# wavelab/libwave

Measured on AMD Instinct MI355X. Metric: point-cloud registrations/sec (1M<->1M pts, ICP), higher is better.
Workload: dtype f32

## Files before the change

### libwave_amd/csrc/wm_nn.hip

```cpp
#include "wm_nn_scan.hpp"

namespace wm {

template <int STATS, bool BAL, bool COST = false>
__global__ void __launch_bounds__(64) __attribute__((amdgpu_waves_per_eu(5, 5)))
    k_nn_grid(const LevelsDev lv, const float4 *__restrict__ src, unsigned n,
              IcpDevState *__restrict__ st, float thr_d2, unsigned long long *__restrict__ keys,
              float4 *__restrict__ match_pt, const float4 *__restrict__ tgt_orig,
              float r_light_cells, float lane_lf, float coop_lf, float r0_cells, unsigned chunk_sz,
              double *__restrict__ partials, unsigned *__restrict__ cost_out,
              unsigned long long *__restrict__ phase_out, long long *__restrict__ bins, float rmax) {
    const unsigned lane = threadIdx.x & 63u;
    const unsigned row_c = xcd_remap_chunked(blockIdx.x, max(chunk_sz, 1u)), row_e = xcd_remap(blockIdx.x, gridDim.x);
    const unsigned row = chunk_sz ? row_c : row_e;
    const unsigned i = row * 64u + lane;
    const bool active = i < n;
    const unsigned ic = min(i, n - 1u);
    const float4 p_e = src[ic];
    const unsigned long long prev_e = keys[ic];
    const float4 tp_e = match_pt[ic];
    const NnState S = nn_state(st);
    const int L = lv.n;
    float hl[kMaxLevels];
#pragma unroll
    for (int k = 0; k < kMaxLevels; ++k) hl[k] = lv.g[k].h;
    asm volatile("" ::WM_NN_STATE_OPERANDS(S), "v"(p_e.x), "v"(p_e.y), "v"(p_e.z), "v"(prev_e), "v"(tp_e.x), "v"(tp_e.y),
                 "v"(tp_e.z), "v"(tp_e.w));
    asm volatile("" ::"s"(L), "s"(hl[0]), "s"(hl[1]), "s"(hl[2]), "s"(hl[3]), "s"(hl[4]), "s"(hl[5]), "s"(r_light_cells),
                 "s"(lane_lf), "s"(r0_cells), "s"(thr_d2), "s"(rmax));
    if (S.done) return;
    unsigned cost = 0;
    unsigned long long prof[3] = {0ull, 0ull, 0ull};
    const unsigned long long prof_start = COST ? clock64() : 0ull;
    __shared__ uint2 s_runs[BAL ? 1 : kRowChunk * 64];
    __shared__ BalHolder<BAL> s_hold;
    const int L_levels = L;
    const float h0 = hl[0];
    const float r_light = r_light_cells * h0;
    const bool have_prev = S.have_prev != 0;
    float qx = 0.f, qy = 0.f, qz = 0.f, r = 0.f;
    float bqx = 0.f, bqy = 0.f, bqz = 0.f;
    unsigned long long best = make_key(thr_d2, kNoIdx);
    unsigned long long seeded = best;
    bool heavy = false;
    bool mine = active;
    unsigned long long prev = ~0ull;
    float4 tp = make_float4(0.f, 0.f, 0.f, 0.f);
    if (active) {
        if (have_prev) {
            prev = prev_e;
            tp = tp_e;
        }
        xform(S.Tf, p_e, qx, qy, qz);
        if (S.slab_on && !(qx >= S.slab_lo && qx < S.slab_hi)) mine = false;
    }
    if (mine) {
        r = r0_cells * h0;
        if (prev != ~0ull) {
            const unsigned pidx = (unsigned) prev;
            r = rmax;
            if (pidx != kNoIdx) {
                const float d2b = canon_d2(qx, qy, qz, tp);
                if (d2b <= thr_d2) {
                    best = seeded = make_key(d2b, pidx);
                    bqx = tp.x;
                    bqy = tp.y;
                    bqz = tp.z;
                    r = fmaxf(__builtin_amdgcn_sqrtf(d2b) * 1.0001f + 1e-6f, 0.05f * h0);
                }
            }
        }
        r = fminf(r, rmax);
        heavy = r > r_light;
    }
    const unsigned long long prof_pro = COST ? clock64() : 0ull;
    if constexpr (BAL) {
        BalLds &L = s_hold.v;
        L.q[lane] = make_float4(qx, qy, qz, 0.f);
        L.seeded[lane] = seeded;
        L.bq[0][lane] = bqx;
        L.bq[1][lane] = bqy;
        L.bq[2][lane] = bqz;
        asm volatile("" ::: "memory");
        bool live = mine && !heavy;
        const bool allow_layered = true;
        for (int pass = 0; pass < 32 && __ballot(live) != 0ull; ++pass) {
            const int l = nn_level_for(hl, L_levels, lane_lf, r);
            const unsigned long long lv_mask = __ballot(live);
            const int l0 = __builtin_amdgcn_readlane(l, __ffsll((long long) lv_mask) - 1);
            float margin;
            if (__ballot(live && l != l0) == 0ull) {
                const GridDev g = lv.g[l0];
                best = scan_box_bal<COST, kBalRowChunk>(g, live, qx, qy, qz, r, best, &margin, L, lane, allow_layered, g.pts, cost, prof);
            } else {
                const GridDev g = lv.g[l];
                L.base[lane] = (unsigned long long) g.pts;
                best = scan_box_bal<COST, kBalRowChunk>(g, live, qx, qy, qz, r, best, &margin, L, lane, allow_layered, nullptr, cost, prof);
            }
            if (live) {
                if constexpr (COST) cost += 1u << 24;
                const float bd2 = __uint_as_float((unsigned) (best >> 32));
                if (nn_certified(margin, bd2, thr_d2)) {
                    live = false;
                } else {
                    r = nn_grow_radius(best, bd2, r, rmax);
                    heavy = r > r_light;
                    live = !heavy;
                }
            }
        }
    } else if (mine) {
        for (int pass = 0; !heavy && pass < 32; ++pass) {
            const int l = nn_level_for(hl, L_levels, lane_lf, r);
            const GridDev g = lv.g[l];
            float margin;
            best = scan_box<COST>(g, qx, qy, qz, r, best, &margin, s_runs, lane, have_prev, cost);
            if constexpr (COST) cost += 1u << 24;
            const float bd2 = __uint_as_float((unsigned) (best >> 32));
            if (nn_certified(margin, bd2, thr_d2)) break;
            r = nn_grow_radius(best, bd2, r, rmax);
            heavy = r > r_light;
        }
    }
    const unsigned long long prof_pass = COST ? clock64() : 0ull;
    unsigned long long todo = __ballot(heavy);
    const unsigned n_heavy = __popcll(todo);
    float seed = 0.f;
    while (todo) {
        const int sl = __ffsll((long long) todo) - 1;
        todo &= todo - 1;
        const float ux = rl_f(qx, sl), uy = rl_f(qy, sl), uz = rl_f(qz, sl);
        float ur = rl_f(r, sl);
        unsigned long long ub = ((unsigned long long) rl_u((unsigned) (best >> 32), sl) << 32) |
                                rl_u((unsigned) best, sl);
        if ((unsigned) ub == kNoIdx && seed > ur) ur = fminf(seed, rmax);
        for (int pass = 0; pass < 64; ++pass) {
            const int l = nn_level_for(hl, L_levels, coop_lf, ur);
            const GridDev g = lv.g[l];
            float margin;
            ub = coop_scan_box(g, ux, uy, uz, ur, ub, lane, &margin);
            const float bd2 = __uint_as_float((unsigned) (ub >> 32));
            if (nn_certified(margin, bd2, thr_d2)) break;
            if (ur >= rmax) break;
            ur = nn_grow_radius(ub, bd2, ur, rmax);
        }
        seed = ((unsigned) ub != kNoIdx) ? 1.25f * sqrtf(__uint_as_float((unsigned) (ub >> 32))) : ur;
        if ((int) lane == sl) best = ub;
    }
    const unsigned lane_e = __builtin_amdgcn_mbcnt_hi(~0u, __builtin_amdgcn_mbcnt_lo(~0u, 0u));
    const unsigned i_e = BAL ? row * 64u + lane_e : i;
    if constexpr (BAL) {
        asm volatile("" ::: "memory");
        BalLds &L = s_hold.v;
        seeded = L.seeded[lane_e];
        bqx = L.bq[0][lane_e];
        bqy = L.bq[1][lane_e];
        bqz = L.bq[2][lane_e];
    }
    if (mine) {
        st_u64(&keys[i_e], best);
        if (best != seeded && (unsigned) best != kNoIdx) {
            const f4v c = ((gp_f4) tgt_orig)[(unsigned) best];
            bqx = c.x;
            bqy = c.y;
            bqz = c.z;
        }
        if (!(best == seeded && (unsigned) best != kNoIdx))
            st_f4(&match_pt[i_e], bqx, bqy, bqz, __uint_as_float((unsigned) best));
    }
    if (lane == 0 && n_heavy) atomicAdd(&st->queue_count[1], n_heavy);
    const unsigned long long prof_store = COST ? clock64() : 0ull;
    if constexpr (COST) {
        if (active) cost_out[i_e] = mine ? (cost | (heavy ? 0x80000000u : 0u)) : 0u;
    }
    if constexpr (STATS >= 0) {
        double a[kAcc];
        icp_terms<STATS>(a, mine, (unsigned) best != kNoIdx, qx, qy, qz, bqx, bqy, bqz,
                         __uint_as_float((unsigned) (best >> 32)),
                         (unsigned) best != (unsigned) seeded && (i_e & st->changed_mask) == 0u);
        acc_halve<kAcc, 32>(a, lane);
        const int comp = acc_comp_of_lane(lane);
        if (comp >= 0) {
            if (bins) bins_add(bins, row % (unsigned) kBinCount, (unsigned) comp, a[0]);
            else st_f64(&partials[(size_t) row * kAcc + comp], a[0]);
        }
    }
    if constexpr (COST) {
        if (lane_e == 0 && phase_out) {
            const unsigned long long t_end = clock64();
            atomicAdd(&phase_out[0], prof[0]);
            atomicAdd(&phase_out[1], prof[1]);
            atomicAdd(&phase_out[2], prof[2]);
            atomicAdd(&phase_out[3], prof_pro - prof_start);
            atomicAdd(&phase_out[4], prof_pass - prof_pro);
            atomicAdd(&phase_out[5], prof_store - prof_pass);
            atomicAdd(&phase_out[6], t_end - prof_store);
            atomicAdd(&phase_out[7], 1ull);
        }
    }
}

constexpr int kBruteTile = 1024;

__global__ void __launch_bounds__(kBlock) k_init_keys(unsigned long long *keys, unsigned n,
                                                       const IcpDevState *st, float thr_d2) {
    if (st->done) return;
    const unsigned i = blockIdx.x * kBlock + threadIdx.x;
    if (i < n) keys[i] = make_key(thr_d2, kNoIdx);
}

__global__ void __launch_bounds__(kBlock)
    k_nn_brute(const float4 *__restrict__ tgt, unsigned m, const float4 *__restrict__ src,
               unsigned n, const IcpDevState *__restrict__ st, float thr_d2,
               unsigned long long *__restrict__ keys) {
    if (st->done) return;
    __shared__ float4 tile[kBruteTile];
    const unsigned i = blockIdx.x * kBlock + threadIdx.x;
    const unsigned per = (m + gridDim.y - 1) / gridDim.y;
    const unsigned m0 = blockIdx.y * per, m1 = min(m0 + per, m);
    float qx = 0, qy = 0, qz = 0;
    if (i < n) xform(st->Tf, src[i], qx, qy, qz);
    const bool mine = !(st->slab_on && !(qx >= st->slab_lo && qx < st->slab_hi));
    unsigned long long best = make_key(thr_d2, kNoIdx);
    for (unsigned t0 = m0; t0 < m1; t0 += kBruteTile) {
        const unsigned cnt = min((unsigned) kBruteTile, m1 - t0);
        __syncthreads();
        for (unsigned k = threadIdx.x; k < cnt; k += kBlock) tile[k] = tgt[t0 + k];
        __syncthreads();
        for (unsigned k = 0; k < cnt; ++k) {
            const float4 t = tile[k];
            const unsigned long long key = make_key(canon_d2(qx, qy, qz, t), __float_as_uint(t.w));
            best = key < best ? key : best;
        }
    }
    if (i < n && mine && best < make_key(thr_d2, kNoIdx)) atomicMin(&keys[i], best);
}

__global__ void __launch_bounds__(kBlock)
    k_fill_match(const unsigned long long *__restrict__ keys, unsigned n,
                 const float4 *__restrict__ tgt, const IcpDevState *__restrict__ st,
                 float4 *__restrict__ match_pt) {
    if (st->done) return;
    const unsigned i = blockIdx.x * kBlock + threadIdx.x;
    if (i >= n) return;
    const unsigned idx = (unsigned) keys[i];
    match_pt[i] = idx == kNoIdx ? make_float4(0.f, 0.f, 0.f, __uint_as_float(kNoIdx)) : tgt[idx];
}

static float threshold_below(double max_corr, bool strict) {
    const double m2 = max_corr * max_corr;
    if (!(m2 < 3.0e38)) return 3.0e38f;
    float f = (float) m2;
    if (strict ? (double) f >= m2 : (double) f > m2) f = nextafterf(f, 0.0f);
    return f;
}
float threshold_d2(double max_corr) { return threshold_below(max_corr, false); }
float threshold_d2_strict(double max_corr) { return threshold_below(max_corr, true); }

int nn_sums_target(wm_ctx *ctx, int stats_mode, bool use_bins, unsigned blocks, long long **bins, unsigned *rows_out) {
    *bins = nullptr;
    if (stats_mode >= 0 && use_bins) {
        if (!ctx->bins.p) return WM_ERR_STATE;
        *bins = ctx->bins.as<long long>();
    } else if (stats_mode >= 0) {
        WM_HIP(ctx, ctx->partials.reserve((size_t) blocks * kAcc * sizeof(double)));
        if (rows_out) *rows_out = blocks;
    }
    return WM_OK;
}

template <int STATS, bool BAL, bool COST = false>
static void launch_nn_grid_t(wm_ctx *ctx, unsigned blocks, float thr_d2, unsigned xcd_chunk, long long *bins = nullptr) {
    hipLaunchKernelGGL(HIP_KERNEL_NAME(k_nn_grid<STATS, BAL, COST>), dim3(blocks), dim3(64), 0, ctx->stream,
                       ctx->levels_dev, ctx->src_sorted.as<float4>(), (unsigned) ctx->n_src,
                       ctx->d_state.as<IcpDevState>(), thr_d2, ctx->keys.as<unsigned long long>(),
                       ctx->match_pt.as<float4>(), ctx->tgt_orig.as<float4>(), ctx->tune_r_light,
                       ctx->tune_lane_lf, ctx->tune_coop_lf, ctx->tune_r0, xcd_chunk, ctx->partials.as<double>(),
                       ctx->cost_log.p ? ctx->cost_log.as<unsigned>() + (size_t) ctx->cost_log_iter * ctx->n_src : nullptr,
                       ctx->phase_log.p ? ctx->phase_log.as<unsigned long long>() + 8 * (size_t) ctx->cost_log_iter : nullptr, bins,
                       sqrtf(thr_d2) * 1.0001f + 1e-6f);
}

int launch_nn_grid(wm_ctx *ctx, float thr_d2, hipEvent_t ev0, hipEvent_t ev1, hipEvent_t ev2,
                   int stats_mode, unsigned *rows_out, bool use_bins) {
    const unsigned n = (unsigned) ctx->n_src;
    if (rows_out) *rows_out = 0;
    if (n == 0) return WM_OK;
    unsigned blocks = (n + 63u) / 64u;
    blocks = (blocks + 7u) & ~7u;
    unsigned xcd_chunk = 0;
    if (ctx->tune_xcd_chunk > 0 && blocks >= 32u * (unsigned) ctx->tune_xcd_chunk) {
        xcd_chunk = (unsigned) ctx->tune_xcd_chunk;
        const unsigned m = 8u * xcd_chunk;
        blocks = (blocks + m - 1u) / m * m;
    }
    long long *bins = nullptr;
    const int rc = nn_sums_target(ctx, stats_mode, use_bins, blocks, &bins, rows_out);
    if (rc != WM_OK) return rc;
    const bool bal = ctx->tune_nn_balanced && ctx->n_tgt_input < (1u << 26) - 8u;
    if (ev0) WM_HIP(ctx, hipEventRecord(ev0, ctx->stream));
    if (stats_mode == WM_ICP_SVD && ctx->cost_log.p && ctx->cost_log_iter < ctx->cost_log_cap) {
        if (bal) launch_nn_grid_t<WM_ICP_SVD, true, true>(ctx, blocks, thr_d2, xcd_chunk, bins);
        else launch_nn_grid_t<WM_ICP_SVD, false, true>(ctx, blocks, thr_d2, xcd_chunk, bins);
        ctx->cost_log_iter++;
    } else if (stats_mode < 0) {
        if (bal) launch_nn_grid_t<-1, true>(ctx, blocks, thr_d2, xcd_chunk);
        else launch_nn_grid_t<-1, false>(ctx, blocks, thr_d2, xcd_chunk);
    } else if (stats_mode == WM_ICP_SVD) {
        if (bal) launch_nn_grid_t<WM_ICP_SVD, true>(ctx, blocks, thr_d2, xcd_chunk, bins);
        else launch_nn_grid_t<WM_ICP_SVD, false>(ctx, blocks, thr_d2, xcd_chunk, bins);
    } else {
        if (bal) launch_nn_grid_t<WM_ICP_GN6, true>(ctx, blocks, thr_d2, xcd_chunk, bins);
        else launch_nn_grid_t<WM_ICP_GN6, false>(ctx, blocks, thr_d2, xcd_chunk, bins);
    }
    if (ev1) WM_HIP(ctx, hipEventRecord(ev1, ctx->stream));
    if (ev2) WM_HIP(ctx, hipEventRecord(ev2, ctx->stream));
    WM_HIP(ctx, hipGetLastError());
    return WM_OK;
}

int launch_nn_brute(wm_ctx *ctx, float thr_d2, hipEvent_t ev0, hipEvent_t ev1) {
    const unsigned n = (unsigned) ctx->n_src, m = (unsigned) ctx->n_tgt_input;
    if (n == 0) return WM_OK;
    const IcpDevState *st = ctx->d_state.as<IcpDevState>();
    unsigned long long *keys = ctx->keys.as<unsigned long long>();
    const unsigned bx = (n + kBlock - 1) / kBlock;
    unsigned splits = 1;
    if (m > 0) {
        splits = (2048 + bx - 1) / bx;
        const unsigned max_splits = (m + kBruteTile - 1) / kBruteTile;
        if (splits > max_splits) splits = max_splits;
        if (splits < 1) splits = 1;
    }
    if (ev0) WM_HIP(ctx, hipEventRecord(ev0, ctx->stream));
    hipLaunchKernelGGL(k_init_keys, dim3(bx), dim3(kBlock), 0, ctx->stream, keys, n, st, thr_d2);
    if (m > 0)
        hipLaunchKernelGGL(k_nn_brute, dim3(bx, splits), dim3(kBlock), 0, ctx->stream,
                           ctx->tgt_orig.as<float4>(), m, ctx->src_sorted.as<float4>(), n, st,
                           thr_d2, keys);
    hipLaunchKernelGGL(k_fill_match, dim3(bx), dim3(kBlock), 0, ctx->stream, keys, n,
                       ctx->tgt_orig.as<float4>(), st, ctx->match_pt.as<float4>());
    if (ev1) WM_HIP(ctx, hipEventRecord(ev1, ctx->stream));
    WM_HIP(ctx, hipGetLastError());
    return WM_OK;
}

}
```

### libwave_amd/csrc/wm_nn_scan.hpp

```cpp
#pragma once
#include "wm_internal.hpp"
#include "wm_icp_step.hpp"
#include "wm_bins.hpp"
#include "wm_wave.hpp"
#include "wm_zigzag.hpp"

namespace wm {

__device__ __forceinline__ unsigned long long make_key(float d2, unsigned idx) {
    return ((unsigned long long) __float_as_uint(d2) << 32) | idx;
}

__device__ __forceinline__ float canon_d2(float qx, float qy, float qz, const float4 &t) {
    const float dx = qx - t.x, dy = qy - t.y, dz = qz - t.z;
    return __fadd_rn(__fadd_rn(__fmul_rn(dx, dx), __fmul_rn(dy, dy)), __fmul_rn(dz, dz));
}

__device__ __forceinline__ void xform(const float *T, const float4 &p, float &x, float &y,
                                      float &z) {
    x = __fadd_rn(__fadd_rn(__fadd_rn(__fmul_rn(T[0], p.x), __fmul_rn(T[1], p.y)),
                            __fmul_rn(T[2], p.z)), T[3]);
    y = __fadd_rn(__fadd_rn(__fadd_rn(__fmul_rn(T[4], p.x), __fmul_rn(T[5], p.y)),
                            __fmul_rn(T[6], p.z)), T[7]);
    z = __fadd_rn(__fadd_rn(__fadd_rn(__fmul_rn(T[8], p.x), __fmul_rn(T[9], p.y)),
                            __fmul_rn(T[10], p.z)), T[11]);
}

__device__ __forceinline__ unsigned xcd_remap(unsigned b, unsigned nblocks) {
    const unsigned per = (nblocks + 7u) / 8u;
    return (b & 7u) * per + (b >> 3);
}
__device__ __forceinline__ unsigned xcd_remap_chunked(unsigned b, unsigned S) {
    const unsigned x = b & 7u, l = b >> 3;
    const unsigned chunk = l / S;
    return (chunk * 8u + x) * S + (l - chunk * S);
}

struct NnState {
    float Tf[12];
    int done, have_prev, slab_on;
    float slab_lo, slab_hi;
    unsigned changed_mask;
    float step_disp;
};
__device__ __forceinline__ NnState nn_state(const IcpDevState *st) {
    NnState s;
#pragma unroll
    for (int k = 0; k < 12; ++k) s.Tf[k] = st->Tf[k];
    s.done = st->done;
    s.have_prev = st->have_prev;
    s.slab_on = st->slab_on;
    s.slab_lo = st->slab_lo;
    s.slab_hi = st->slab_hi;
    s.changed_mask = st->changed_mask;
    s.step_disp = st->step_disp;
    return s;
}
#define WM_NN_STATE_OPERANDS(s)                                                                                              \
    "s"((s).Tf[0]), "s"((s).Tf[1]), "s"((s).Tf[2]), "s"((s).Tf[3]), "s"((s).Tf[4]), "s"((s).Tf[5]), "s"((s).Tf[6]),           \
        "s"((s).Tf[7]), "s"((s).Tf[8]), "s"((s).Tf[9]), "s"((s).Tf[10]), "s"((s).Tf[11]), "s"((s).done), "s"((s).have_prev), \
        "s"((s).slab_on), "s"((s).slab_lo), "s"((s).slab_hi)

typedef float f4v __attribute__((ext_vector_type(4)));
typedef const __attribute__((address_space(1))) f4v *gp_f4;
typedef const __attribute__((address_space(1))) unsigned *gp_u32;
__device__ __forceinline__ float4 ldp(const float4 *p, size_t j) {
    const f4v v = ((gp_f4) p)[j];
    return make_float4(v.x, v.y, v.z, v.w);
}
__device__ __forceinline__ unsigned ldc(const unsigned *p, size_t j) { return ((gp_u32) p)[j]; }
__device__ __forceinline__ void st_f4(float4 *p, float x, float y, float z, float w) {
    f4v v = {x, y, z, w};
    __builtin_nontemporal_store(v, (f4v *) p);
}
__device__ __forceinline__ void st_u64(unsigned long long *p, unsigned long long v) { __builtin_nontemporal_store(v, p); }
__device__ __forceinline__ void st_f64(double *p, double v) { __builtin_nontemporal_store(v, p); }
__device__ __forceinline__ float canon_d2v(float qx, float qy, float qz, const f4v &t) {
    return canon_d2(qx, qy, qz, make_float4(t.x, t.y, t.z, t.w));
}

__device__ __forceinline__ unsigned long long scan_run(const float4 *__restrict__ pts, unsigned s,
                                                       unsigned e, float qx, float qy, float qz,
                                                       unsigned long long best) {
    for (unsigned j = s; j < e; j += 4) {
        const gp_f4 p = (gp_f4) pts + j;
        const f4v t0 = p[0], t1 = p[1], t2 = p[2], t3 = p[3];
        const unsigned long long k0 = make_key(canon_d2v(qx, qy, qz, t0), __float_as_uint(t0.w));
        const unsigned long long k1 = make_key(canon_d2v(qx, qy, qz, t1), __float_as_uint(t1.w));
        const unsigned long long k2 = make_key(canon_d2v(qx, qy, qz, t2), __float_as_uint(t2.w));
        const unsigned long long k3 = make_key(canon_d2v(qx, qy, qz, t3), __float_as_uint(t3.w));
        const unsigned long long a = k0 < k1 ? k0 : k1, b = k2 < k3 ? k2 : k3;
        const unsigned long long m = a < b ? a : b;
        best = m < best ? m : best;
    }
    return best;
}

constexpr int kRowChunk = 6;
constexpr int kLayeredRows = 18;
template <bool COST>
__device__ __forceinline__ unsigned long long scan_box(const GridDev &g, float qx, float qy,
                                                       float qz, float r, unsigned long long best,
                                                       float *margin, uint2 *runs, unsigned lane,
                                                       bool allow_layered, unsigned &cost) {
    const float big = 4.0e6f;
    const float fx = fminf(fmaxf((qx - g.ox) * g.inv_h, -big), big);
    const float fy = fminf(fmaxf((qy - g.oy) * g.inv_h, -big), big);
    const float fz = fminf(fmaxf((qz - g.oz) * g.inv_h, -big), big);
    const float rc = r * g.inv_h + g.slack;
    const int x0 = (int) floorf(fx - rc), x1 = (int) floorf(fx + rc);
    const int y0 = (int) floorf(fy - rc), y1 = (int) floorf(fy + rc);
    const int z0 = (int) floorf(fz - rc), z1 = (int) floorf(fz + rc);
    const float mx = fminf(fx - (float) x0, (float) (x1 + 1) - fx);
    const float my = fminf(fy - (float) y0, (float) (y1 + 1) - fy);
    const float mz = fminf(fz - (float) z0, (float) (z1 + 1) - fz);
    *margin = (fminf(mx, fminf(my, mz)) - g.slack) * g.h;
    const int xa = max(x0, 0), xb = min(x1, g.nx - 1);
    const int ya = max(y0, 0), yb = min(y1, g.ny - 1);
    const int za = max(z0, 0), zb = min(z1, g.nz - 1);
    if (xa > xb || ya > yb || za > zb) return best;
    auto lookup_and_walk = [&](const unsigned (&a0)[kRowChunk], const unsigned (&a1)[kRowChunk]) {
        unsigned rs[kRowChunk], re[kRowChunk];
#pragma unroll
        for (int u = 0; u < kRowChunk; ++u) {
            rs[u] = ldc(g.cell_start, a0[u]);
            re[u] = ldc(g.cell_start, a1[u]);
        }
        unsigned cnt = 0;
        if constexpr (COST) cost += 1u << 16;
#pragma unroll
        for (int u = 0; u < kRowChunk; ++u)
            if (re[u] > rs[u]) runs[cnt++ * 64u + lane] = make_uint2(rs[u], re[u]);
        unsigned idx = 0, j = 0, e = 0;
        if (cnt) {
            const uint2 run = runs[lane];
            j = run.x;
            e = run.y;
        }
        while (j < e) {
            const gp_f4 p = (gp_f4) g.pts + j;
            const f4v t0 = p[0], t1 = p[1], t2 = p[2], t3 = p[3];
            const unsigned long long k0 = make_key(canon_d2v(qx, qy, qz, t0), __float_as_uint(t0.w));
            const unsigned long long k1 = make_key(canon_d2v(qx, qy, qz, t1), __float_as_uint(t1.w));
            const unsigned long long k2 = make_key(canon_d2v(qx, qy, qz, t2), __float_as_uint(t2.w));
            const unsigned long long k3 = make_key(canon_d2v(qx, qy, qz, t3), __float_as_uint(t3.w));
            const unsigned long long a = k0 < k1 ? k0 : k1, b = k2 < k3 ? k2 : k3;
            const unsigned long long m = a < b ? a : b;
            best = m < best ? m : best;
            j += 4;
            if constexpr (COST) cost += 1u;
            if (j >= e && ++idx < cnt) {
                const uint2 run = runs[idx * 64u + lane];
                j = run.x;
                e = run.y;
            }
        }
    };
    const bool layered =
        allow_layered && __popcll(__ballot((yb - ya + 1) * (zb - za + 1) > kLayeredRows)) >= 8;
    if (layered) {
        for (int kz = 0;; ++kz) {
            const int zz = za + kz;
            const bool zact = zz <= zb;
            if (__ballot(zact) == 0ull) break;
            const float Rb =
                __builtin_amdgcn_sqrtf(__uint_as_float((unsigned) (best >> 32))) * g.inv_h * 1.00001f;
            const float lim = Rb + g.slack;
            const float lim2 = lim * lim, c0 = Rb * Rb + 2.f * g.slack * lim;
            const float rz = fmaxf(fmaxf((float) zz - fz, fz - (float) (zz + 1)), 0.f);
            const float rz2 = rz * rz;
            const float hy = __builtin_amdgcn_sqrtf(fmaxf(lim2 - rz2, 0.f)) * 1.00001f;
            const bool zin = zact && !(rz2 > lim2);
            const int yl = zin ? max(ya, __float2int_rd(fy - hy)) : 1;
            const int yh = zin ? min(yb, __float2int_rd(fy + hy)) : 0;
            const unsigned basez = (unsigned) zz * g.ny * g.nx;
            for (int y0 = yl; __ballot(y0 <= yh) != 0ull; y0 += kRowChunk) {
                unsigned a0[kRowChunk], a1[kRowChunk];
#pragma unroll
                for (int u = 0; u < kRowChunk; ++u) {
                    const int yy = y0 + u;
                    const float yf = (float) yy;
                    const float ry = fmaxf(fmaxf(yf - fy, fy - (yf + 1.f)), 0.f);
                    const float rho2 = ry * ry + rz2;
                    const float hx = __builtin_amdgcn_sqrtf(fmaxf(c0 - rho2, 0.f)) * 1.00001f + g.slack;
                    const int xl = max(xa, __float2int_rd(fx - hx)), xh = min(xb, __float2int_rd(fx + hx));
                    const bool ok = yy <= yh && !(rho2 > lim2) && xl <= xh;
                    const unsigned base = basez + (unsigned) yy * g.nx;
                    a0[u] = ok ? base + xl : 0u;
                    a1[u] = ok ? base + xh + 1 : 0u;
                }
                lookup_and_walk(a0, a1);
            }
        }
        return best;
    }
    int yy = ya, zz = za;
    while (zz <= zb) {
        const float Rb =
            __builtin_amdgcn_sqrtf(__uint_as_float((unsigned) (best >> 32))) * g.inv_h * 1.00001f;
        const float lim = Rb + g.slack;
        const float lim2 = lim * lim, c0 = Rb * Rb + 2.f * g.slack * lim;
        unsigned a0[kRowChunk], a1[kRowChunk];
#pragma unroll
        for (int u = 0; u < kRowChunk; ++u) {
            const float ry = fmaxf(fmaxf((float) yy - fy, fy - (float) (yy + 1)), 0.f);
            const float rz = fmaxf(fmaxf((float) zz - fz, fz - (float) (zz + 1)), 0.f);
            const float rho2 = ry * ry + rz * rz;
            const float hx = __builtin_amdgcn_sqrtf(fmaxf(c0 - rho2, 0.f)) * 1.00001f + g.slack;
            const int xl = max(xa, __float2int_rd(fx - hx)), xh = min(xb, __float2int_rd(fx + hx));
            const bool ok = zz <= zb && !(rho2 > lim2) && xl <= xh;
            const unsigned base = ((unsigned) zz * g.ny + yy) * g.nx;
            a0[u] = ok ? base + xl : 0u;
            a1[u] = ok ? base + xh + 1 : 0u;
            const bool wrap = yy >= yb;
            yy = wrap ? ya : yy + 1;
            zz += wrap;
        }
        lookup_and_walk(a0, a1);
    }
    return best;
}

__device__ __forceinline__ unsigned long long scan_run_bound(const float4 *__restrict__ pts, unsigned s, unsigned e,
                                                             float qx, float qy, float qz, unsigned long long best,
                                                             unsigned &second) {
    for (unsigned j = s; j < e; j += 4) {
        const gp_f4 p = (gp_f4) pts + j;
        const f4v t[4] = {p[0], p[1], p[2], p[3]};
#pragma unroll
        for (int u = 0; u < 4; ++u) {
            const unsigned long long k = make_key(canon_d2v(qx, qy, qz, t[u]), __float_as_uint(t[u].w));
            if (k < best) {
                second = min(second, (unsigned) (best >> 32));
                best = k;
            } else if (k != best) {
                second = min(second, (unsigned) (k >> 32));
            }
        }
    }
    return best;
}

__device__ __forceinline__ unsigned long long wave_min_u64(unsigned long long v) {
#pragma unroll
    for (int off = 32; off > 0; off >>= 1) {
        const unsigned long long o = __shfl_xor(v, off);
        v = o < v ? o : v;
    }
    return v;
}

__device__ __forceinline__ float rl_f(float v, int lane) {
    return __int_as_float(__builtin_amdgcn_readlane(__float_as_int(v), lane));
}
__device__ __forceinline__ unsigned rl_u(unsigned v, int lane) {
    return (unsigned) __builtin_amdgcn_readlane((int) v, lane);
}

constexpr int kBalCap = 1024;
constexpr int kBalRowChunk = 3;
struct BalLds {
    unsigned items[kBalCap + 1];
    float4 q[64];
    unsigned long long base[64];
    unsigned long long best[64];
    unsigned long long seeded[64];
    float bq[3][64];
};

__device__ __forceinline__ unsigned wave_incl_scan(unsigned v) {
    v += (unsigned) __builtin_amdgcn_update_dpp(0, (int) v, 0x111, 0xf, 0xf, true);
    v += (unsigned) __builtin_amdgcn_update_dpp(0, (int) v, 0x112, 0xf, 0xf, true);
    v += (unsigned) __builtin_amdgcn_update_dpp(0, (int) v, 0x114, 0xf, 0xf, true);
    v += (unsigned) __builtin_amdgcn_update_dpp(0, (int) v, 0x118, 0xf, 0xf, true);
    v += (unsigned) __builtin_amdgcn_update_dpp(0, (int) v, 0x142, 0xa, 0xf, false);
    v += (unsigned) __builtin_amdgcn_update_dpp(0, (int) v, 0x143, 0xc, 0xf, false);
    return v;
}

template <bool B>
struct BalHolder {
    BalLds v;
};
template <>
struct BalHolder<false> {
    int unused;
};

struct Bound {
    unsigned second;
    float pad;
    unsigned *lds;
    float4 *win;
    bool ok;
    __device__ __forceinline__ float prune_r(unsigned long long best) const {
        const float b = __builtin_amdgcn_sqrtf(__uint_as_float((unsigned) (best >> 32))) * 1.00001f + pad;
        return fminf(b, __builtin_amdgcn_sqrtf(__uint_as_float(second)) * 1.00001f);
    }
};

template <bool BOUND>
__device__ __forceinline__ void pooled_rounds(BalLds &L, const unsigned *items, unsigned T, unsigned lane,
                                              const float4 *ubase, Bound *bnd) {
    for (unsigned k0 = 0; k0 < T; k0 += 64u) {
        const unsigned k = k0 + lane;
        if (k < T) {
            const unsigned it = items[k];
            const unsigned owner = it >> 26, j = it & 0x3FFFFFFu;
            const float4 q = L.q[owner];
            const gp_f4 p = (gp_f4) (ubase ? ubase : (const float4 *) L.base[owner]) + j;
            const f4v t0 = p[0], t1 = p[1], t2 = p[2], t3 = p[3];
            const float d0 = canon_d2v(q.x, q.y, q.z, t0), d1 = canon_d2v(q.x, q.y, q.z, t1);
            const float d2 = canon_d2v(q.x, q.y, q.z, t2), d3 = canon_d2v(q.x, q.y, q.z, t3);
            const unsigned m = min(min(__float_as_uint(d0), __float_as_uint(d1)), min(__float_as_uint(d2), __float_as_uint(d3)));
            if (m <= __float_as_uint(q.w)) {
                const unsigned long long k0_ = make_key(d0, __float_as_uint(t0.w)), k1_ = make_key(d1, __float_as_uint(t1.w));
                const unsigned long long k2_ = make_key(d2, __float_as_uint(t2.w)), k3_ = make_key(d3, __float_as_uint(t3.w));
                const unsigned long long a = k0_ < k1_ ? k0_ : k1_, b = k2_ < k3_ ? k2_ : k3_;
                if constexpr (BOUND) {
                    const unsigned long long mn = a < b ? a : b;
                    const unsigned u0 = __float_as_uint(d0), u1 = __float_as_uint(d1), u2 = __float_as_uint(d2),
                                   u3 = __float_as_uint(d3);
                    const unsigned lo01 = min(u0, u1), hi01 = max(u0, u1), lo23 = min(u2, u3), hi23 = max(u2, u3);
                    const unsigned sec = min(max(lo01, lo23), min(hi01, hi23));
                    const unsigned long long old = atomicMin(&L.best[owner], mn);
                    unsigned push = sec;
                    if (old != mn) push = min(push, (unsigned) ((old > mn ? old : mn) >> 32));
                    atomicMin(&bnd->lds[owner], push);
                    if (old > mn && bnd->win) {
                        const f4v c = mn == k0_ ? t0 : (mn == k1_ ? t1 : (mn == k2_ ? t2 : t3));
                        bnd->win[owner] = make_float4(c.x, c.y, c.z, c.w);
                    }
                } else {
                    atomicMin(&L.best[owner], a < b ? a : b);
                }
            }
        }
    }
}

template <bool COST, int RC, bool BOUND = false>
__device__ __forceinline__ void balanced_walk(BalLds &L, const unsigned (&rs)[RC],
                                              const unsigned (&re)[RC], unsigned lane,
                                              const float4 *pts, const float4 *ubase, float qx, float qy,
                                              float qz, unsigned long long &best, unsigned &cost,
                                              unsigned long long *prof, Bound *bnd = nullptr) {
    const unsigned long long prof_t0 = COST ? clock64() : 0ull;
    unsigned len[RC], t = 0, longest = 0;
#pragma unroll
    for (int u = 0; u < RC; ++u) {
        len[u] = (unsigned) max((int) (re[u] - rs[u]), 0);
        t += (len[u] + 3u) >> 2;
        longest = max(longest, len[u]);
    }
    const unsigned incl = wave_incl_scan(t);
    const unsigned T = rl_u(incl, 63);
    if (T == 0u) return;
    if constexpr (COST) cost += t;
    if (T > (unsigned) kBalCap) {
        if constexpr (BOUND) {
#pragma unroll
            for (int u = 0; u < RC; ++u) best = scan_run_bound(pts, rs[u], re[u], qx, qy, qz, best, bnd->second);
        } else {
#pragma unroll
            for (int u = 0; u < RC; ++u) best = scan_run(pts, rs[u], re[u], qx, qy, qz, best);
        }
        return;
    }
    unsigned off = incl - t;
    const unsigned tag = lane << 26;
    if (__ballot(longest > 8u) == 0ull) {
#pragma unroll
        for (int u = 0; u < RC; ++u) {
            L.items[len[u] > 0u ? off : (unsigned) kBalCap] = tag | rs[u];
            L.items[len[u] > 4u ? off + 1u : (unsigned) kBalCap] = tag | (rs[u] + 4u);
            off += (len[u] + 3u) >> 2;
        }
    } else {
#pragma unroll
        for (int u = 0; u < RC; ++u)
            for (unsigned j = rs[u]; j < re[u]; j += 4u) L.items[off++] = tag | j;
    }
    L.best[lane] = best;
    if constexpr (BOUND) {
        const float pr = bnd->prune_r(best);
        bnd->lds[lane] = bnd->second;
        reinterpret_cast<unsigned *>(&L.q[lane])[3] = __float_as_uint(pr * pr);
    } else {
        reinterpret_cast<unsigned *>(&L.q[lane])[3] = (unsigned) (best >> 32);
    }
    __builtin_amdgcn_wave_barrier();
    pooled_rounds<BOUND>(L, L.items, T, lane, ubase, bnd);
    __builtin_amdgcn_wave_barrier();
    best = L.best[lane];
    if constexpr (BOUND) bnd->second = bnd->lds[lane];
    if constexpr (COST) {
        prof[0] += clock64() - prof_t0;
        prof[1] += (T + 63u) / 64u;
        prof[2] += 1;
    }
}

template <bool COST, int RC, bool BOUND = false>
__device__ __forceinline__ unsigned long long scan_box_bal(const GridDev &g, bool live, float qx, float qy,
                                                           float qz, float r, unsigned long long best,
                                                           float *margin, BalLds &L, unsigned lane,
                                                           bool allow_layered, const float4 *ubase,
                                                           unsigned &cost, unsigned long long *prof, Bound *bnd = nullptr) {
    const float big = 4.0e6f;
    const float fx = fminf(fmaxf((qx - g.ox) * g.inv_h, -big), big);
    const float fy = fminf(fmaxf((qy - g.oy) * g.inv_h, -big), big);
    const float fz = fminf(fmaxf((qz - g.oz) * g.inv_h, -big), big);
    const float rc = r * g.inv_h + g.slack;
    const int x0 = (int) floorf(fx - rc), x1 = (int) floorf(fx + rc);
    const int y0 = (int) floorf(fy - rc), y1 = (int) floorf(fy + rc);
    const int z0 = (int) floorf(fz - rc), z1 = (int) floorf(fz + rc);
    const float mx = fminf(fx - (float) x0, (float) (x1 + 1) - fx);
    const float my = fminf(fy - (float) y0, (float) (y1 + 1) - fy);
    const float mz = fminf(fz - (float) z0, (float) (z1 + 1) - fz);
    *margin = (fminf(mx, fminf(my, mz)) - g.slack) * g.h;
    const int xa = max(x0, 0), xb = min(x1, g.nx - 1);
    const int ya = max(y0, 0), yb = min(y1, g.ny - 1);
    const int za = max(z0, 0), zb = min(z1, g.nz - 1);
    const bool has = live && !(xa > xb || ya > yb || za > zb);
    auto lookup_and_walk = [&](const unsigned (&a0)[RC], const unsigned (&a1)[RC]) {
        unsigned rs[RC], re[RC];
#pragma unroll
        for (int u = 0; u < RC; ++u) {
            rs[u] = ldc(g.cell_start, a0[u]);
            re[u] = ldc(g.cell_start, a1[u]);
        }
        if constexpr (COST) cost += has ? 1u << 16 : 0u;
        balanced_walk<COST, RC, BOUND>(L, rs, re, lane, g.pts, ubase, qx, qy, qz, best, cost, prof, bnd);
    };
    auto ball_r = [&]() -> float {
        if constexpr (BOUND) return bnd->prune_r(best) * g.inv_h * 1.00001f;
        else return __builtin_amdgcn_sqrtf(__uint_as_float((unsigned) (best >> 32))) * g.inv_h * 1.00001f;
    };
    const bool layered =
        allow_layered && __popcll(__ballot(has && (yb - ya + 1) * (zb - za + 1) > kLayeredRows)) >= 8;
    if (layered) {
        const int zq = min(max(__float2int_rd(fz), za), zb);
        for (int kz = 0;; ++kz) {
            const float Rb = ball_r();
            const float lim = Rb + g.slack;
            const float lim2 = lim * lim;
            const float dz = zigzag_remaining(kz, za, zq, zb, 0.f);
            const bool zact = has && kz <= zb - za && !(dz * dz > lim2);
            if (__ballot(zact) == 0ull) break;
            const int zz = zigzag_coord(kz, za, zq, zb);
            const float rz = fmaxf(fmaxf((float) zz - fz, fz - (float) (zz + 1)), 0.f);
            const float rz2 = rz * rz;
            const float hy = __builtin_amdgcn_sqrtf(fmaxf(lim2 - rz2, 0.f)) * 1.00001f;
            const bool zin = zact && !(rz2 > lim2);
            const int yl = zin ? max(ya, __float2int_rd(fy - hy)) : 1;
            const int yh = zin ? min(yb, __float2int_rd(fy + hy)) : 0;
            const int yc = min(max(__float2int_rd(fy), yl), yh);
            const unsigned basez = (unsigned) zz * g.ny * g.nx;
            for (int ky = 0;; ky += RC) {
                const float Rc = ball_r();
                const float limc = Rc + g.slack;
                const float limc2 = limc * limc, c0 = Rc * Rc + 2.f * g.slack * limc;
                const float dy = zigzag_remaining(ky, yl, yc, yh, 0.f);
                const bool yact = ky <= yh - yl && !(dy * dy + rz2 > limc2);
                if (__ballot(yact) == 0ull) break;
                unsigned a0[RC], a1[RC];
#pragma unroll
                for (int u = 0; u < RC; ++u) {
                    const int yy = zigzag_coord(ky + u, yl, yc, yh);
                    const float yf = (float) yy;
                    const float ry = fmaxf(fmaxf(yf - fy, fy - (yf + 1.f)), 0.f);
                    const float rho2 = ry * ry + rz2;
                    const float hx = __builtin_amdgcn_sqrtf(fmaxf(c0 - rho2, 0.f)) * 1.00001f + g.slack;
                    const int xl = max(xa, __float2int_rd(fx - hx)), xh = min(xb, __float2int_rd(fx + hx));
                    const bool ok = yact && ky + u <= yh - yl && !(rho2 > limc2) && xl <= xh;
                    const unsigned base = basez + (unsigned) yy * g.nx;
                    a0[u] = ok ? base + xl : 0u;
                    a1[u] = ok ? base + xh + 1 : 0u;
                }
                lookup_and_walk(a0, a1);
            }
        }
        return best;
    }
    int yy = ya, zz = has ? za : zb + 1;
    while (__ballot(zz <= zb) != 0ull) {
        const float Rb = ball_r();
        const float lim = Rb + g.slack;
        const float lim2 = lim * lim, c0 = Rb * Rb + 2.f * g.slack * lim;
        unsigned a0[RC], a1[RC];
#pragma unroll
        for (int u = 0; u < RC; ++u) {
            const float ry = fmaxf(fmaxf((float) yy - fy, fy - (float) (yy + 1)), 0.f);
            const float rz = fmaxf(fmaxf((float) zz - fz, fz - (float) (zz + 1)), 0.f);
            const float rho2 = ry * ry + rz * rz;
            const float hx = __builtin_amdgcn_sqrtf(fmaxf(c0 - rho2, 0.f)) * 1.00001f + g.slack;
            const int xl = max(xa, __float2int_rd(fx - hx)), xh = min(xb, __float2int_rd(fx + hx));
            const bool ok = zz <= zb && !(rho2 > lim2) && xl <= xh;
            const unsigned base = ((unsigned) zz * g.ny + yy) * g.nx;
            a0[u] = ok ? base + xl : 0u;
            a1[u] = ok ? base + xh + 1 : 0u;
            const bool wrap = yy >= yb;
            yy = wrap ? ya : yy + 1;
            zz += (wrap && zz <= zb) ? 1 : 0;
        }
        lookup_and_walk(a0, a1);
    }
    return best;
}

constexpr unsigned kRowPool = 128, kRowsPerLane = 16, kRowTrips = 512;
struct RowLds {
    unsigned trips[kRowTrips];
    unsigned map[kRowPool];
    int box[5][64];
};
static_assert(sizeof(RowLds) <= sizeof(unsigned) * (kBalCap + 1), "RowLds overlays BalLds::items");

__device__ __forceinline__ bool scan_box_rows(const GridDev &g, bool live, float qx, float qy, float qz, float r,
                                              unsigned long long &best, float *margin, BalLds &L, unsigned lane,
                                              Bound *bnd) {
    const float big = 4.0e6f;
    const float fx = fminf(fmaxf((qx - g.ox) * g.inv_h, -big), big);
    const float fy = fminf(fmaxf((qy - g.oy) * g.inv_h, -big), big);
    const float fz = fminf(fmaxf((qz - g.oz) * g.inv_h, -big), big);
    const float rc = r * g.inv_h + g.slack;
    const int x0 = (int) floorf(fx - rc), x1 = (int) floorf(fx + rc);
    const int y0 = (int) floorf(fy - rc), y1 = (int) floorf(fy + rc);
    const int z0 = (int) floorf(fz - rc), z1 = (int) floorf(fz + rc);
    const int xa = max(x0, 0), xb = min(x1, g.nx - 1);
    const int ya = max(y0, 0), yb = min(y1, g.ny - 1);
    const int za = max(z0, 0), zb = min(z1, g.nz - 1);
    const bool has = live && !(xa > xb || ya > yb || za > zb);
    const int wy = yb - ya + 1;
    const unsigned nrows = has ? (unsigned) (wy * (zb - za + 1)) : 0u;
    const unsigned incl = wave_incl_scan(nrows);
    const unsigned R = rl_u(incl, 63);
    if (R > kRowPool || __ballot(nrows > kRowsPerLane) != 0ull) return false;
    {
        const float mx = fminf(fx - (float) x0, (float) (x1 + 1) - fx);
        const float my = fminf(fy - (float) y0, (float) (y1 + 1) - fy);
        const float mz = fminf(fz - (float) z0, (float) (z1 + 1) - fz);
        *margin = (fminf(mx, fminf(my, mz)) - g.slack) * g.h;
    }
    if (R == 0u) return true;
    RowLds &W = *reinterpret_cast<RowLds *>(L.items);
    const float pr = bnd->prune_r(best);
    L.best[lane] = best;
    bnd->lds[lane] = bnd->second;
    reinterpret_cast<unsigned *>(&L.q[lane])[3] = __float_as_uint(pr * pr);
    W.box[0][lane] = xa;
    W.box[1][lane] = xb;
    W.box[2][lane] = ya;
    W.box[3][lane] = za;
    W.box[4][lane] = wy;
    for (unsigned k = 0, off = incl - nrows; k < nrows; ++k) W.map[off + k] = lane | (k << 8);
    __builtin_amdgcn_wave_barrier();
    unsigned ttot = 0;
    bool fits = true;
    for (unsigned b0 = 0; b0 < R; b0 += 64u) {
        unsigned rs = 0, re = 0, owner = 0;
        if (b0 + lane < R) {
            const unsigned m = W.map[b0 + lane];
            owner = m & 63u;
            const int k = (int) (m >> 8), wyo = W.box[4][owner];
            const int yy = W.box[2][owner] + k % wyo, zz = W.box[3][owner] + k / wyo;
            const float4 q = L.q[owner];
            const float ofx = fminf(fmaxf((q.x - g.ox) * g.inv_h, -big), big);
            const float ofy = fminf(fmaxf((q.y - g.oy) * g.inv_h, -big), big);
            const float ofz = fminf(fmaxf((q.z - g.oz) * g.inv_h, -big), big);
            const float Rb = __builtin_amdgcn_sqrtf(q.w) * g.inv_h * 1.00003f;
            const float lim = Rb + g.slack;
            const float lim2 = lim * lim, c0 = Rb * Rb + 2.f * g.slack * lim;
            const float ry = fmaxf(fmaxf((float) yy - ofy, ofy - (float) (yy + 1)), 0.f);
            const float rz = fmaxf(fmaxf((float) zz - ofz, ofz - (float) (zz + 1)), 0.f);
            const float rho2 = ry * ry + rz * rz;
            const float hx = __builtin_amdgcn_sqrtf(fmaxf(c0 - rho2, 0.f)) * 1.00001f + g.slack;
            const int xl = max(W.box[0][owner], __float2int_rd(ofx - hx)), xh = min(W.box[1][owner], __float2int_rd(ofx + hx));
            if (!(rho2 > lim2) && xl <= xh) {
                const unsigned base = ((unsigned) zz * g.ny + yy) * g.nx;
                rs = ldc(g.cell_start, base + xl);
                re = ldc(g.cell_start, base + xh + 1);
            }
        }
        const unsigned len = (unsigned) max((int) (re - rs), 0), t = (len + 3u) >> 2;
        const unsigned incl2 = wave_incl_scan(t);
        const unsigned Tb = rl_u(incl2, 63);
        if (Tb > kRowTrips) {
            fits = false;
            break;
        }
        if (ttot + Tb > kRowTrips) {
            __builtin_amdgcn_wave_barrier();
            pooled_rounds<true>(L, W.trips, ttot, lane, g.pts, bnd);
            __builtin_amdgcn_wave_barrier();
            ttot = 0;
        }
        unsigned o = ttot + incl2 - t;
        for (unsigned j = rs; j < re; j += 4u) W.trips[o++] = (owner << 26) | j;
        ttot += Tb;
    }
    __builtin_amdgcn_wave_barrier();
    if (fits) pooled_rounds<true>(L, W.trips, ttot, lane, g.pts, bnd);
    __builtin_amdgcn_wave_barrier();
    best = L.best[lane];
    bnd->second = bnd->lds[lane];
    return fits;
}

__device__ __forceinline__ unsigned long long coop_scan_box(const GridDev &g, float qx, float qy,
                                                            float qz, float r,
                                                            unsigned long long best, unsigned lane,
                                                            float *margin, unsigned *second_out = nullptr,
                                                            float pad = 0.f) {
    const float fx = (qx - g.ox) * g.inv_h, fy = (qy - g.oy) * g.inv_h, fz = (qz - g.oz) * g.inv_h;
    const float rc = r * g.inv_h + g.slack;
    const float big = 4.0e6f;
    const int x0 = (int) floorf(fminf(fmaxf(fx - rc, -big), big));
    const int x1 = (int) floorf(fminf(fmaxf(fx + rc, -big), big));
    const int y0 = (int) floorf(fminf(fmaxf(fy - rc, -big), big));
    const int y1 = (int) floorf(fminf(fmaxf(fy + rc, -big), big));
    const int z0 = (int) floorf(fminf(fmaxf(fz - rc, -big), big));
    const int z1 = (int) floorf(fminf(fmaxf(fz + rc, -big), big));
    const float mx = fminf(fx - (float) x0, (float) (x1 + 1) - fx);
    const float my = fminf(fy - (float) y0, (float) (y1 + 1) - fy);
    const float mz = fminf(fz - (float) z0, (float) (z1 + 1) - fz);
    *margin = (fminf(mx, fminf(my, mz)) - g.slack) * g.h;
    const int xa = max(x0, 0), xb = min(x1, g.nx - 1);
    const int ya = max(y0, 0), yb = min(y1, g.ny - 1);
    const int za = max(z0, 0), zb = min(z1, g.nz - 1);
    if (xa > xb || ya > yb || za > zb) return best;
    const int cy = (int) floorf(fminf(fmaxf(fy, -big), big));
    const int cz = (int) floorf(fminf(fmaxf(fz, -big), big));
    const int wy = yb - ya + 1;
    const int nrows = wy * (zb - za + 1);
    const float bd2 = __uint_as_float((unsigned) (best >> 32));
    const float Rb = (__builtin_amdgcn_sqrtf(bd2) + pad) * g.inv_h * 1.00001f;
    unsigned long long mine = best;
    unsigned mine2 = 0x7F800000u;
    for (int k0 = 0; k0 < nrows; k0 += 64) {
        const int k = k0 + (int) lane;
        unsigned s = 0, e = 0;
        if (k < nrows) {
            const int yy = ya + k % wy, zz = za + k / wy;
            const float ry = yy > cy ? (float) yy - fy : (yy < cy ? fy - (float) (yy + 1) : 0.f);
            const float rz = zz > cz ? (float) zz - fz : (zz < cz ? fz - (float) (zz + 1) : 0.f);
            const float rho2 = ry * ry + rz * rz;
            const float lim = Rb + g.slack;
            if (!(rho2 > lim * lim)) {
                const float hx2 = fmaxf(Rb * Rb - rho2 + 2.f * g.slack * lim, 0.f);
                const float hx = __builtin_amdgcn_sqrtf(hx2) * 1.00001f + g.slack;
                const int xl = max(xa, (int) floorf(fminf(fmaxf(fx - hx, -big), big)));
                const int xh = min(xb, (int) floorf(fminf(fmaxf(fx + hx, -big), big)));
                if (xl <= xh) {
                    const size_t base = ((size_t) zz * g.ny + yy) * g.nx;
                    s = ldc(g.cell_start, base + xl);
                    e = ldc(g.cell_start, base + xh + 1);
                }
            }
        }
        unsigned long long rows = __ballot(e > s);
        while (rows) {
            const int rl = __ffsll((long long) rows) - 1;
            rows &= rows - 1;
            const unsigned rs = rl_u(s, rl), re = rl_u(e, rl);
            for (unsigned j = rs + lane; j < re; j += 128u) {
                const float4 t0 = ldp(g.pts, j);
                const float4 t1 = ldp(g.pts, j + 64u < re ? j + 64u : j);
                const unsigned long long a = make_key(canon_d2(qx, qy, qz, t0), __float_as_uint(t0.w));
                const unsigned long long b = make_key(canon_d2(qx, qy, qz, t1), __float_as_uint(t1.w));
                const unsigned long long m = a < b ? a : b;
                if (second_out) {
                    const unsigned long long hi = a < b ? b : a;
                    if (m < mine) {
                        mine2 = min(mine2, min((unsigned) (mine >> 32), hi != m ? (unsigned) (hi >> 32) : 0x7F800000u));
                    } else {
                        if (m != mine) mine2 = min(mine2, (unsigned) (m >> 32));
                        if (hi != mine && hi != m) mine2 = min(mine2, (unsigned) (hi >> 32));
                    }
                }
                mine = m < mine ? m : mine;
            }
        }
    }
    const unsigned long long all = wave_min_u64(mine);
    if (second_out) {
        unsigned v = mine != all ? min(mine2, (unsigned) (mine >> 32)) : mine2;
#pragma unroll
        for (int off = 32; off > 0; off >>= 1) v = min(v, (unsigned) __shfl_xor((int) v, off));
        *second_out = min(*second_out, v);
    }
    return all;
}

__device__ __forceinline__ bool nn_certified(float margin, float bd2, float thr_d2) {
    return margin > 0.f && (bd2 <= margin * margin || thr_d2 <= margin * margin);
}
__device__ __forceinline__ float nn_grow_radius(unsigned long long best, float bd2, float r, float rmax, float pad = 0.f) {
    const float rn = ((unsigned) best != kNoIdx) ? __builtin_amdgcn_sqrtf(bd2) * 1.0001f + 1e-6f + pad : 2.0f * r;
    return fminf(fmaxf(rn, 1.25f * r), rmax);
}
__device__ __forceinline__ int nn_level_for(const float (&hl)[kMaxLevels], int levels, float lf, float r) {
    int l = 0;
#pragma unroll
    for (int k = 0; k < kMaxLevels - 1; ++k) l += (k < levels - 1 && hl[k] < lf * r) ? 1 : 0;
    return l;
}
constexpr int kCertWaves = 4;
__device__ __forceinline__ void chunk_query(unsigned e, const unsigned (&cum)[kCertWaves + 1], unsigned &w, unsigned &k) {
    w = (e >= cum[1] ? 1u : 0u) + (e >= cum[2] ? 1u : 0u) + (e >= cum[3] ? 1u : 0u);
    k = e - (w == 0u ? cum[0] : (w == 1u ? cum[1] : (w == 2u ? cum[2] : cum[3])));
}
__device__ __forceinline__ double add_wave_rows(const double (&rows)[kCertWaves][kAcc], unsigned c) {
    double t = rows[0][c];
#pragma unroll
    for (int w = 1; w < kCertWaves; ++w) t += rows[w][c];
    return t;
}


constexpr double kChangedUnit = 1.0 / 16777216.0;
template <int STATS>
__device__ __forceinline__ void icp_terms(double (&a)[kAcc], bool mine, bool matched, float qx, float qy, float qz,
                                          float bqx, float bqy, float bqz, float d2, bool changed = false) {
#pragma unroll
    for (int k = 0; k < kAcc; ++k) a[k] = 0.0;
    if (mine) {
        a[17] = changed ? 1.0 + kChangedUnit : 1.0;
        if (matched) {
            const double px = qx, py = qy, pz = qz, tx = bqx, ty = bqy, tz = bqz;
            a[0] = 1.0;
            a[1] = px;
            a[2] = py;
            a[3] = pz;
            if constexpr (STATS == WM_ICP_SVD) {
                a[4] = tx;
                a[5] = ty;
                a[6] = tz;
                a[7] = tx * px;
                a[8] = tx * py;
                a[9] = tx * pz;
                a[10] = ty * px;
                a[11] = ty * py;
                a[12] = ty * pz;
                a[13] = tz * px;
                a[14] = tz * py;
                a[15] = tz * pz;
            } else {
                const double rx = px - tx, ry = py - ty, rz = pz - tz;
                a[4] = py * py + pz * pz;
                a[5] = -px * py;
                a[6] = -px * pz;
                a[7] = px * px + pz * pz;
                a[8] = -py * pz;
                a[9] = px * px + py * py;
                a[10] = rx;
                a[11] = ry;
                a[12] = rz;
                a[13] = py * rz - pz * ry;
                a[14] = pz * rx - px * rz;
                a[15] = px * ry - py * rx;
            }
            a[16] = (double) d2;
        }
    }
}

}
```

Before: 290.6.

## Add emptiness-probe ladder to seed unseeded queries before balanced NN scan

For lanes with no prior match, the balanced path now runs a doubling-radius probe that checks cell-range occupancy only (no point distance scans). On the first non-empty box it picks a middle point as a candidate and tightens the search radius; empty boxes grow the radius directly. The aim is to avoid expensive full box scans at radii that are too small or too large for unseeded queries. It adds extra cell_start loads and wave-wide loops, and the r_light value is recomputed through an opaque lambda, apparently to influence register allocation. The cost counters are also saturated.

After: 295.0 (median of 6 runs). 1.01x the previous value.

```diff
diff --git a/libwave_amd/csrc/wm_nn.hip b/libwave_amd/csrc/wm_nn.hip
--- a/libwave_amd/csrc/wm_nn.hip
+++ b/libwave_amd/csrc/wm_nn.hip
@@ -36,7 +36,11 @@
     __shared__ BalHolder<BAL> s_hold;
     const int L_levels = L;
     const float h0 = hl[0];
-    const float r_light = r_light_cells * h0;
+    auto r_light = [&]() -> float {
+        float c = r_light_cells;
+        asm volatile("" : "+s"(c));
+        return c * h0;
+    };
     const bool have_prev = S.have_prev != 0;
     float qx = 0.f, qy = 0.f, qz = 0.f, r = 0.f;
     float bqx = 0.f, bqy = 0.f, bqz = 0.f;
@@ -71,7 +75,7 @@
             }
         }
         r = fminf(r, rmax);
-        heavy = r > r_light;
+        heavy = r > r_light();
     }
     const unsigned long long prof_pro = COST ? clock64() : 0ull;
     if constexpr (BAL) {
@@ -84,6 +88,38 @@
         asm volatile("" ::: "memory");
         bool live = mine && !heavy;
         const bool allow_layered = true;
+        bool probing = live && (unsigned) best == kNoIdx && r < rmax;
+        if (__ballot(probing) != 0ull) {
+            float rp = r0_cells * h0;
+            for (int rung = 0; rung < 16 && __ballot(probing) != 0ull; ++rung) {
+                int lp = 0;
+#pragma unroll
+                for (int k = 1; k < kMaxLevels; ++k) lp += (k < L_levels && hl[k] <= rp) ? 1 : 0;
+                const GridDev g = lv.g[lp];
+                unsigned cand;
+                const bool empty = probe_box_empty(g, probing, qx, qy, qz, rp, cand);
+                const bool hit = probing && !empty;
+                const f4v ct = ((gp_f4) g.pts)[hit ? cand : 0u];
+                if (hit) {
+                    const float d2c = canon_d2v(qx, qy, qz, ct);
+                    const float rc = fmaxf(__builtin_amdgcn_sqrtf(d2c) * 1.0001f + 1e-6f, 0.05f * h0);
+                    if (d2c <= thr_d2 && rc <= r_light()) {
+                        best = make_key(d2c, __float_as_uint(ct.w));
+                        r = fminf(rc, rmax);
+                    }
+                }
+                if (probing) {
+                    if constexpr (COST) cost += ((cost >> 28) & 7u) < 7u ? 1u << 28 : 0u;
+                    if (empty) {
+                        r = nn_grow_radius(best, 0.f, r, rmax);
+                        heavy = r > r_light();
+                        live = !heavy;
+                    }
+                    probing = empty && live && r < rmax;
+                }
+                rp = fminf(2.0f * rp, rmax);
+            }
+        }
         for (int pass = 0; pass < 32 && __ballot(live) != 0ull; ++pass) {
             const int l = nn_level_for(hl, L_levels, lane_lf, r);
             const unsigned long long lv_mask = __ballot(live);
@@ -98,13 +134,13 @@
                 best = scan_box_bal<COST, kBalRowChunk>(g, live, qx, qy, qz, r, best, &margin, L, lane, allow_layered, nullptr, cost, prof);
             }
             if (live) {
-                if constexpr (COST) cost += 1u << 24;
+                if constexpr (COST) cost += ((cost >> 24) & 15u) < 15u ? 1u << 24 : 0u;
                 const float bd2 = __uint_as_float((unsigned) (best >> 32));
                 if (nn_certified(margin, bd2, thr_d2)) {
                     live = false;
                 } else {
                     r = nn_grow_radius(best, bd2, r, rmax);
-                    heavy = r > r_light;
+                    heavy = r > r_light();
                     live = !heavy;
                 }
             }
@@ -115,11 +151,11 @@
             const GridDev g = lv.g[l];
             float margin;
             best = scan_box<COST>(g, qx, qy, qz, r, best, &margin, s_runs, lane, have_prev, cost);
-            if constexpr (COST) cost += 1u << 24;
+            if constexpr (COST) cost += ((cost >> 24) & 15u) < 15u ? 1u << 24 : 0u;
             const float bd2 = __uint_as_float((unsigned) (best >> 32));
             if (nn_certified(margin, bd2, thr_d2)) break;
             r = nn_grow_radius(best, bd2, r, rmax);
-            heavy = r > r_light;
+            heavy = r > r_light();
         }
     }
     const unsigned long long prof_pass = COST ? clock64() : 0ull;
diff --git a/libwave_amd/csrc/wm_nn_scan.hpp b/libwave_amd/csrc/wm_nn_scan.hpp
--- a/libwave_amd/csrc/wm_nn_scan.hpp
+++ b/libwave_amd/csrc/wm_nn_scan.hpp
@@ -507,6 +507,68 @@
         lookup_and_walk(a0, a1);
     }
     return best;
+}
+
+constexpr int kProbeRows = 9;
+struct ProbeBox {
+    int xa, xb, ya, yb, zb, yy, zz;
+    unsigned found;
+    unsigned cand;
+    __device__ __forceinline__ ProbeBox(const GridDev &g, bool probing, float qx, float qy, float qz, float r) {
+        const float big = 4.0e6f;
+        const float fx = fminf(fmaxf((qx - g.ox) * g.inv_h, -big), big);
+        const float fy = fminf(fmaxf((qy - g.oy) * g.inv_h, -big), big);
+        const float fz = fminf(fmaxf((qz - g.oz) * g.inv_h, -big), big);
+        const float rc = r * g.inv_h + g.slack;
+        xa = max((int) floorf(fx - rc), 0), xb = min((int) floorf(fx + rc), g.nx - 1);
+        ya = max((int) floorf(fy - rc), 0), yb = min((int) floorf(fy + rc), g.ny - 1);
+        const int za = max((int) floorf(fz - rc), 0);
+        zb = min((int) floorf(fz + rc), g.nz - 1);
+        const bool has = probing && !(xa > xb || ya > yb || za > zb);
+        found = 0u;
+        cand = 0u;
+        yy = ya, zz = has ? za : zb + 1;
+    }
+    __device__ __forceinline__ bool more() const { return zz <= zb && found == 0u; }
+    __device__ __forceinline__ void request(const GridDev &g, unsigned (&rs)[kProbeRows], unsigned (&re)[kProbeRows]) {
+        unsigned a0[kProbeRows], a1[kProbeRows];
+        const bool go = found == 0u;
+#pragma unroll
+        for (int u = 0; u < kProbeRows; ++u) {
+            const bool ok = go && zz <= zb;
+            const unsigned base = ((unsigned) zz * g.ny + yy) * g.nx;
+            a0[u] = ok ? base + xa : 0u;
+            a1[u] = ok ? base + xb + 1 : 0u;
+            const bool wrap = yy >= yb;
+            yy = wrap ? ya : yy + 1;
+            zz += (wrap && zz <= zb) ? 1 : 0;
+        }
+#pragma unroll
+        for (int u = 0; u < kProbeRows; ++u) {
+            rs[u] = ldc(g.cell_start, a0[u]);
+            re[u] = ldc(g.cell_start, a1[u]);
+        }
+    }
+    __device__ __forceinline__ void take(const unsigned (&rs)[kProbeRows], const unsigned (&re)[kProbeRows]) {
+#pragma unroll
+        for (int u = 0; u < kProbeRows; ++u) found |= re[u] - rs[u];
+        const int order[kProbeRows] = {8, 6, 2, 0, 7, 5, 3, 1, 4};
+#pragma unroll
+        for (int k = 0; k < kProbeRows; ++k) {
+            const int u = order[k];
+            if (re[u] != rs[u]) cand = (rs[u] + re[u]) >> 1;
+        }
+    }
+};
+__device__ __forceinline__ bool probe_box_empty(const GridDev &g, bool probing, float qx, float qy, float qz, float r, unsigned &cand) {
+    ProbeBox b(g, probing, qx, qy, qz, r);
+    while (__ballot(b.more()) != 0ull) {
+        unsigned rs[kProbeRows], re[kProbeRows];
+        b.request(g, rs, re);
+        b.take(rs, re);
+    }
+    cand = b.cand;
+    return b.found == 0u;
 }
 
 constexpr unsigned kRowPool = 128, kRowsPerLane = 16, kRowTrips = 512;
```
